# rfonod/geo-trax

Measured on AMD Instinct MI355X. Metric: 4K frames/sec through detect+stabilize+track, higher is better.
Workload: dtype f32 (split-f16x3 MFMA)

## Files before the change

geo-trax_amd/csrc/det_kernels.hip:

```cpp
#include <hip/hip_runtime.h>

#include <mutex>
#include <hip/hip_fp16.h>

#include <cmath>

#include "det_kernels.hpp"

namespace gtx {

typedef _Float16 half8 __attribute__((ext_vector_type(8)));
typedef _Float16 half4 __attribute__((ext_vector_type(4)));

namespace {
inline double py_round(double v) { return std::nearbyint(v); }
}

Letterbox letterbox_geometry(int src_h, int src_w, int imgsz, bool rect, int stride) {
  Letterbox lb{};
  lb.src_h = src_h;
  lb.src_w = src_w;
  const double r = std::min((double)imgsz / src_h, (double)imgsz / src_w);
  lb.new_w = (int)py_round(src_w * r);
  lb.new_h = (int)py_round(src_h * r);
// ... 884 lines not shown
      const float hw = b.z / 2.f, hh = b.w / 2.f;
      reinterpret_cast<float4*>(nb.cand_box)[o] = make_float4(b.x - hw, b.y - hh, b.x + hw, b.y + hh);
    }
  }
}

template <typename T>
__global__ __launch_bounds__(256) void head_raw_kernel(const HeadParams hp, float* __restrict__ out, int logits) {
  const int n = blockIdx.y;
  const int lane = threadIdx.x & 63;
  const int a = (blockIdx.x * blockDim.x + threadIdx.x) >> 6;
  if (a >= hp.n_anchors) return;
  const int l = find_level(hp, a);
  const HeadLevel& L = hp.lv[l];
  const int la = a - L.anchor_begin;
  const T* f = static_cast<const T*>(L.feat) + ((size_t)n * L.h * L.w + la) * L.cstride;
  const float4 b = anchor_box<T>(L, f, la, lane);
  float* o = out + ((size_t)n * hp.n_anchors + a) * (4 + hp.nc);
  if (lane == 0) { o[0] = b.x; o[1] = b.y; o[2] = b.z; o[3] = b.w; }
  const T* fc = f + L.cb;
  for (int c = lane; c < hp.nc; c += 64) {
    float acc = L.bc[c];
    for (int k = 0; k < L.cc; ++k) acc = fmaf(ldf(fc + k), L.wc[c * L.cc + k], acc);
    o[4 + c] = logits ? acc : 1.f / (1.f + expf(-acc));
  }
}

void launch_head_candidates(int dtype, const HeadParams& hp, int n, const NmsBuffers& nb, hipStream_t s) {
  launch_head_gate(dtype, hp, n, nb, s);
  launch_head_boxes(dtype, hp, n, nb, s);
}

void launch_head_gate(int dtype, const HeadParams& hp, int n, const NmsBuffers& nb, hipStream_t s) {
  GTX_HIP(hipMemsetAsync(nb.count, 0, sizeof(int) * n, s));
  if (nb.lvl_count) GTX_HIP(hipMemsetAsync(nb.lvl_count, 0, sizeof(int) * n * kMaxLevels, s));
  dim3 grid(cdiv(hp.n_anchors, 16), n), block(256);
  if (dtype == DT_F16) hipLaunchKernelGGL(head_candidates_kernel<_Float16>, grid, block, 0, s, hp, nb);
  else hipLaunchKernelGGL(head_candidates_kernel<float>, grid, block, 0, s, hp, nb);
  GTX_HIP(hipGetLastError());
}

void launch_head_boxes(int dtype, const HeadParams& hp, int n, const NmsBuffers& nb, hipStream_t s) {
  dim3 grid2(64, n), block(256);
  const size_t lds = (size_t)hp.n_levels * hp.lv[0].cb * 64 * sizeof(float);
  GTX_CHECK(hp.n_levels <= kMaxLevels && hp.lv[0].cb <= 128, "head: %d levels of %d box channels", hp.n_levels, hp.lv[0].cb);
  static std::once_flag once;
  std::call_once(once, [] {
    GTX_HIP(hipFuncSetAttribute(reinterpret_cast<const void*>(head_boxes_kernel<_Float16>), hipFuncAttributeMaxDynamicSharedMemorySize, kMaxLevels * 128 * 64 * 4));
    GTX_HIP(hipFuncSetAttribute(reinterpret_cast<const void*>(head_boxes_kernel<float>), hipFuncAttributeMaxDynamicSharedMemorySize, kMaxLevels * 128 * 64 * 4));
  });
  if (dtype == DT_F16) hipLaunchKernelGGL(head_boxes_kernel<_Float16>, grid2, block, lds, s, hp, nb);
  else hipLaunchKernelGGL(head_boxes_kernel<float>, grid2, block, lds, s, hp, nb);
  GTX_HIP(hipGetLastError());
}

void launch_head_raw(int dtype, const HeadParams& hp, int n, float* out, bool logits, hipStream_t s) {
  dim3 grid(cdiv(hp.n_anchors * 64, 256), n), block(256);
  if (dtype == DT_F16) hipLaunchKernelGGL(head_raw_kernel<_Float16>, grid, block, 0, s, hp, out, logits ? 1 : 0);
  else hipLaunchKernelGGL(head_raw_kernel<float>, grid, block, 0, s, hp, out, logits ? 1 : 0);
  GTX_HIP(hipGetLastError());
}

constexpr int kSmallNms = 4096;
constexpr int kSmallKeep = 2048;

__global__ __launch_bounds__(256) void nms_rank_kernel(const NmsBuffers nb, int limit, float cls_offset) {
  __shared__ float s_sc[256];
  __shared__ int s_an[256];
// ... 146 lines not shown
    if (slot >= nb.max_det) continue;
    float4 b = boxes[i];
    b.x = (b.x - padx) / gain; b.y = (b.y - pady) / gain;
    b.z = (b.z - padx) / gain; b.w = (b.w - pady) / gain;
    b.x = fminf(fmaxf(b.x, 0.f), fw); b.z = fminf(fmaxf(b.z, 0.f), fw);
    b.y = fminf(fmaxf(b.y, 0.f), fh); b.w = fminf(fmaxf(b.w, 0.f), fh);
    float* r = rows + (size_t)slot * 6;
    r[0] = b.x; r[1] = b.y; r[2] = b.z; r[3] = b.w;
    r[4] = nb.s_score[(size_t)n * nb.nms_cap + i];
    r[5] = (float)nb.s_cls[(size_t)n * nb.nms_cap + i];
    if (nb.out_anchor) nb.out_anchor[(size_t)n * nb.max_det + slot] = nb.s_anchor[(size_t)n * nb.nms_cap + i];
  }
}


__device__ __forceinline__ bool iou_gt(const float4& a, float area_a, const float4& b, float thr) {
  const float iw = fminf(a.z, b.z) - fmaxf(a.x, b.x);
  const float ih = fminf(a.w, b.w) - fmaxf(a.y, b.y);
  if (!(iw > 0.f && ih > 0.f)) return false;
  const float area_b = (b.z - b.x) * (b.w - b.y);
  const float inter = iw * ih;
  return inter / (area_a + area_b - inter) > thr;
}

__global__ __launch_bounds__(1024) void nms_small_kernel(const NmsBuffers nb, float thr, float cls_offset, float gain, float padx,
                                                         float pady, float fw, float fh) {
  __shared__ unsigned long long s_key[kSmallNms];
  __shared__ float4 s_box[kSmallNms];
  __shared__ float4 s_kbox[kSmallKeep];
  __shared__ int s_nkeep, s_done;
  const int n = blockIdx.x;
  const int tid = threadIdx.x, lane = tid & 63;
  const int wave = __builtin_amdgcn_readfirstlane(tid >> 6), nwaves = blockDim.x >> 6;
  const int cnt = min(nb.count[n], nb.cap);
  if (cnt > kSmallNms || nb.max_det > kSmallKeep) {
    if (tid == 0) nb.out_n[n] = 0;
    return;
  }
  if (tid == 0) { nb.sorted_n[n] = 0; s_nkeep = 0; s_done = 0; }
  const size_t base = (size_t)n * nb.cap;
  int P = 64;
  while (P < cnt) P <<= 1;
  for (int i = tid; i < P; i += blockDim.x) {
    unsigned long long k = 0ull;
    if (i < cnt) {
      const unsigned sb = __float_as_uint(nb.cand_score[base + i]);
      k = ((unsigned long long)sb << 32) | ((unsigned long long)(0x7FFFFu - (unsigned)nb.cand_anchor[base + i]) << 12) | (unsigned)i;
    }
    s_key[i] = k;
  }
  __syncthreads();
  for (int k = 2; k <= P; k <<= 1)
    for (int j = k >> 1; j > 0; j >>= 1) {
      for (int t = tid; t < P / 2; t += blockDim.x) {
        const int lo = ((t / j) * 2 * j) + (t % j), hi = lo + j;
        const bool desc = ((lo & k) == 0);
        const unsigned long long a = s_key[lo], b = s_key[hi];
        if ((a < b) == desc) { s_key[lo] = b; s_key[hi] = a; }
      }
      __syncthreads();
    }
  for (int i = tid; i < cnt; i += blockDim.x) {
    const int slot = (int)(s_key[i] & 0xFFFu);
    float4 b = reinterpret_cast<const float4*>(nb.cand_box)[base + slot];
    const float o = cls_offset * (float)nb.cand_cls[base + slot];
    b.x += o; b.y += o; b.z += o; b.w += o;
    s_box[i] = b;
// ... 132 lines not shown
```

geo-trax_amd/csrc/det_kernels.hpp:

```cpp
#pragma once
#include <vector>

#include "common.hpp"
#include "conv_igemm.hpp"

namespace gtx {

struct Letterbox {
  int src_h, src_w;
  int net_h, net_w;
  int new_h, new_w;
  int top, left;
  double gain;
};
Letterbox letterbox_geometry(int src_h, int src_w, int imgsz, bool rect, int stride);

void launch_preprocess(int dtype, const uint8_t* frames, int n, const Letterbox& lb, void* img,
                       uint8_t* gray, int gh, int gw, hipStream_t s);

void launch_stem(int dtype, const void* img, int n, int h, int w, const float* w27, const float* bias,
                 const void* wpk_f16, int c0, void* out, int ho, int wo, hipStream_t s, float acc_scale = 1.f);
std::vector<uint16_t> pack_stem_weights_f16(const float* w27, int c0);
std::vector<uint16_t> pack_stem_weights_split(const float* w27, int c0, float* acc_scale);

// ... 14 lines not shown
  float stride;
  int anchor_begin;
};
struct HeadParams {
  HeadLevel lv[kMaxLevels];
  int n_levels;
  int n_anchors;
  int nc;
  float conf;
  unsigned long long class_mask[2];
};

struct NmsBuffers {
  int cap;
  int* count;
  float* cand_score;
  int* cand_anchor;
  int* cand_cls;
  float* cand_box;
  int nms_cap;
  int* sorted_n;
  float* s_box;
  float* s_score;
  int* s_cls;
  int* s_anchor;
  unsigned long long* mask;
  int max_det;
  int* out_n;
  float* out_rows;
  int* out_anchor;
  int* lvl_count;
  int* lvl_list;
  int lvl_cap;
};

struct FeatLevels {
  const void* feat[kMaxLevels];
  int h[kMaxLevels], w[kMaxLevels], cstride[kMaxLevels], coff[kMaxLevels], c[kMaxLevels];
  int anchor_begin[kMaxLevels];
  int n_levels;
  int dim;
};
void launch_obj_feats(int dtype, const FeatLevels& fl, int n, const NmsBuffers& nb, float* out, hipStream_t s);

void launch_head_candidates(int dtype, const HeadParams& hp, int n, const NmsBuffers& nb, hipStream_t s);
void launch_head_gate(int dtype, const HeadParams& hp, int n, const NmsBuffers& nb, hipStream_t s);
void launch_head_boxes(int dtype, const HeadParams& hp, int n, const NmsBuffers& nb, hipStream_t s);

struct SparseBoxLevel {
  const void* in;
  int H, W, cstride, coff, cin;
  const void* w1; const float* b1; float sc1;
  const void* w2; const float* b2; float sc2;
  int anchor_begin;
  const float* wb; const float* bb; float stride;
};
struct SparseBox {
  SparseBoxLevel lv[kMaxLevels];
  int n_levels;
  int cap;
  int* sat_flag;
};
void launch_head_sparse_box(const SparseBox& sb, int n, const NmsBuffers& nb, hipStream_t s);
constexpr int kV10Keep = 300;
void launch_v10_select(int dtype, const HeadParams& hp, int n, const NmsBuffers& cand, const NmsBuffers& sel, float* scores, hipStream_t s);
void launch_v10_rows(const NmsBuffers& sel, const unsigned long long class_mask[2], int n, const Letterbox& lb, hipStream_t s);
// ... 7 lines not shown
```

geo-trax_amd/csrc/detector.cpp:

```cpp
#include "detector.hpp"
#include "split_format.hpp"

#include <algorithm>
#include <cmath>

namespace gtx {

Detector::Detector(gtx_ctx* ctx, const gtx_det_config& cfg)
    : DetectorBase(ctx, cfg, cfg.half ? DT_F16 : (cfg.fp32_split ? DT_F32S : DT_F32), dtype_size(cfg.half ? DT_F16 : DT_F32),
                   cfg.half ? DT_F16 : DT_F32),
      trunk_(*this, ops_, cfg.half ? DT_F16 : DT_F32) {
  dtype_ = cfg.half ? DT_F16 : DT_F32;
  es_ = dtype_size(dtype_);
  lb_ = letterbox_geometry(cfg.frame_h, cfg.frame_w, cfg.imgsz, cfg.rect != 0, 32);
  GTX_CHECK(lb_.net_h % 32 == 0 && lb_.net_w % 32 == 0, "network input %dx%d is not stride aligned", lb_.net_h, lb_.net_w);
}

Detector::~Detector() {
  if (h_feats_) (void)hipHostFree(h_feats_);
  if (h_count_) (void)hipHostFree(h_count_);
}

std::unique_ptr<NetRuntime> Detector::make_exact() const {
  gtx_det_config c = cfg_;
  c.fp32_split = 0;
  return std::unique_ptr<NetRuntime>(new Detector(ctx_, c));
}

View Detector::head_conv(const std::string& name, const View& x, const View* out_slice) {
  ConvArgs a;
  a.out_slice = out_slice;
  a.plain_out = fmt_ == DT_F32S && plain_out_;
  a.force_kc = force_kc_; a.force_bn = force_bn_;
  return emit_named_conv(ops_, name, x, a);
}

void Detector::build_graph() {
  const int H = lb_.net_h, W = lb_.net_w;
  img_ = new_view(H, W, 4);
  alloc_sat_flag();
  const YoloTrunk::Levels trunk = trunk_.build(img_);
  const std::vector<View>& lvl_in = trunk.in;
  const std::vector<float>& strides = trunk.strides;
  det_pfx_ = trunk.det_pfx;
  const int nl = (int)lvl_in.size();
  GTX_CHECK(nl <= kMaxLevels, "internal: %d Detect levels", nl);
  const bool has_o2o = has(det_pfx_ + ".one2one_cv2.0.0.conv.weight");
  end2end_ = cfg_.end2end != 0;
  GTX_CHECK(!end2end_ || has_o2o, "end2end: the checkpoint has no one-to-one head (%s.one2one_cv2 / one2one_cv3): only a YOLOv10 file has", det_pfx_.c_str());
  GTX_CHECK(!end2end_ || !cfg_.obj_feats, "end2end: obj_feats (ReID `model: auto`) is not implemented for the one-to-one head");
  const std::string box_br = end2end_ ? ".one2one_cv2." : ".cv2.", cls_br = end2end_ ? ".one2one_cv3." : ".cv3.";
  GTX_CHECK(has(det_pfx_ + box_br + "0.0.conv.weight") && has(det_pfx_ + cls_br + "0.2.weight"),
            "%s: the checkpoint holds no %s / %s tensors (a fused YOLOv10 export keeps the one-to-one head only: run it with end2end)", det_pfx_.c_str(),
            box_br.substr(1, box_br.size() - 2).c_str(), cls_br.substr(1, cls_br.size() - 2).c_str());

  std::vector<Op> st1, st2;
  const bool dw_cls = trunk.dw_cls;
  std::vector<Op> dw_a, pw_a, dw_b;
  head_ = HeadParams{};
  head_.n_levels = nl;
  head_.nc = cfg_.nc;
  head_.conf = cfg_.conf;
  head_.class_mask[0] = head_.class_mask[1] = cfg_.n_classes == 0 ? ~0ull : 0ull;
  for (int i = 0; i < cfg_.n_classes; ++i)
    if (cfg_.classes[i] >= 0 && cfg_.classes[i] < 128) head_.class_mask[cfg_.classes[i] >> 6] |= 1ull << (cfg_.classes[i] & 63);
  int anchor = 0;
  for (int l = 0; l < nl; ++l) {
    const std::string b2 = det_pfx_ + box_br + std::to_string(l), b3 = det_pfx_ + cls_br + std::to_string(l);
    const HostTensor &w20 = tensor(b2 + ".0.conv.weight"), &w30 = tensor(b3 + (dw_cls ? ".1.1.conv.weight" : ".0.conv.weight"));
    const int cb = (int)w20.shape[0], cc = (int)w30.shape[0], cin = (int)w20.shape[1];
    GTX_CHECK(cin == lvl_in[l].c && (dw_cls || (int)w30.shape[1] == cin), "Detect level %d input channels", l);
    Op o1, o2, o3;
    View h2;
// ... 261 lines not shown
  }
}

void Detector::prime_pad_skip() {
  if (pad_skip_rows_ == 0) return;
  const int N = cfg_.max_batch;
  hipStream_t s = ctx_->stream;
  DevBuf blank;
  blank.alloc((size_t)N * cfg_.frame_h * cfg_.frame_w * 3);
  GTX_HIP(hipMemsetAsync(blank.p, 0, blank.bytes, s));
  pad_skip_on_ = false;
  cur_nb_ = 0;
  set_batch(N);
  launch_preprocess(dtype_, (const uint8_t*)blank.p, N, lb_, img_.ptr, nullptr, cfg_.frame_h / 2, cfg_.frame_w / 2, s);
  for (const Op& op : ops_) run_op(op, N, s);
  int sat = 0;
  if (sat_dev_) GTX_HIP(hipMemcpyAsync(&sat, sat_dev_, sizeof(int), hipMemcpyDeviceToHost, s));
  GTX_HIP(hipStreamSynchronize(s));
  cur_nb_ = 0;
  if (sat_dev_) GTX_HIP(hipMemsetAsync(sat_dev_, 0, sizeof(int), s));
  if (sat) {
    pad_skip_on_ = false;
    pad_skip_rows_ = 0;
    for (Op& op : ops_)
      for (int i = 0; i < kMaxGroup; ++i) op.ty_first[i] = op.ty_count[i] = 0;
    return;
  }
  pad_skip_on_ = true;
}

void Detector::finalize() {
  GTX_CHECK(!finalized_, "finalize called twice");
  GTX_HIP(hipSetDevice(ctx_->device));
  build_graph();
  trunk_.fuse();
  const int N = cfg_.max_batch;
  alloc_outputs();
  nms_ = NmsBuffers{};
  nms_.cap = head_.n_anchors;
  nms_.nms_cap = 30016;
  nms_.max_det = cfg_.max_det;
  nms_.count = (int*)alloc(sizeof(int) * N);
  nms_.cand_score = (float*)alloc(sizeof(float) * N * nms_.cap);
  nms_.cand_anchor = (int*)alloc(sizeof(int) * N * nms_.cap);
  nms_.cand_cls = (int*)alloc(sizeof(int) * N * nms_.cap);
  nms_.cand_box = (float*)alloc(sizeof(float) * 4 * N * nms_.cap);
  if (!end2end_) {
    nms_.sorted_n = (int*)alloc(sizeof(int) * N);
    nms_.s_box = (float*)alloc(sizeof(float) * 4 * N * nms_.nms_cap);
    nms_.s_score = (float*)alloc(sizeof(float) * N * nms_.nms_cap);
    nms_.s_cls = (int*)alloc(sizeof(int) * N * nms_.nms_cap);
    nms_.mask = (unsigned long long*)alloc(sizeof(unsigned long long) * N * (size_t)nms_.nms_cap * (nms_.nms_cap / 64));
  }
  nms_.out_n = (int*)alloc(sizeof(int) * N);
  nms_.out_rows = (float*)alloc(sizeof(float) * 6 * N * cfg_.max_det);
  nms_.s_anchor = nms_.out_anchor = nullptr;
  if (cfg_.obj_feats) {
    nms_.s_anchor = (int*)alloc(sizeof(int) * N * nms_.nms_cap);
    nms_.out_anchor = (int*)alloc(sizeof(int) * N * cfg_.max_det);
    d_feats_ = (float*)alloc(sizeof(float) * N * cfg_.max_det * feat_levels_.dim);
    GTX_HIP(hipHostMalloc((void**)&h_feats_, sizeof(float) * N * cfg_.max_det * feat_levels_.dim));
  }
  if (sparse_on_ && !end2end_) {
    sparse_.cap = kSparseCap;
    sparse_.sat_flag = sat_dev_;
    nms_.lvl_cap = kSparseCap;
    nms_.lvl_count = (int*)alloc(sizeof(int) * N * kMaxLevels);
    nms_.lvl_list = (int*)alloc(sizeof(int) * N * kMaxLevels * kSparseCap);
  }
  if (end2end_) {
    sel_ = nms_;
    sel_.cap = kSelCap;
    sel_.count = (int*)alloc(sizeof(int) * N);
    sel_.cand_score = (float*)alloc(sizeof(float) * N * kSelCap);
    sel_.cand_anchor = (int*)alloc(sizeof(int) * N * kSelCap);
    sel_.cand_cls = (int*)alloc(sizeof(int) * N * kSelCap);
    sel_.cand_box = (float*)alloc(sizeof(float) * 4 * N * kSelCap);
    sel_.lvl_count = sel_.lvl_list = nullptr;
    sel_.lvl_cap = 0;
    if (sparse_on_) {
      sparse_.cap = kSelCap;
      sparse_.sat_flag = sat_dev_;
      sel_.lvl_cap = kSelCap;
      sel_.lvl_count = (int*)alloc(sizeof(int) * N * kMaxLevels);
      sel_.lvl_list = (int*)alloc(sizeof(int) * N * kMaxLevels * kSelCap);
    }
    v10_scores_ = (float*)alloc(sizeof(float) * N * kV10Keep * cfg_.nc);
  }
  GTX_HIP(hipHostMalloc((void**)&h_count_, sizeof(int) * N));
  drop_tensors_unless_fallback();
  if (env_flag("GTX_PAD_SKIP", true)) {
    plan_pad_skip();
    prime_pad_skip();
  }
  set_batch(1);
  GTX_HIP(hipStreamSynchronize(ctx_->stream));
  finalized_ = true;
}

void Detector::run_op(const Op& op, int nb, hipStream_t s) { trunk_.run_op(op, nb, s); }

void Detector::run_post(int nb, hipStream_t s) {
  if (end2end_) {
    HeadParams gate = head_;
    gate.class_mask[0] = gate.class_mask[1] = ~0ull;
    launch_head_gate(dtype_, gate, nb, nms_, s);
    launch_v10_select(dtype_, head_, nb, nms_, sel_, v10_scores_, s);
    if (sparse_on_) {
      launch_head_sparse_box(sparse_, nb, sel_, s);
      dense_head_valid_ = false;
    } else {
      launch_head_boxes(dtype_, head_, nb, sel_, s);
    }
    launch_v10_rows(sel_, head_.class_mask, nb, lb_, s);
    GTX_HIP(hipMemcpyAsync(h_count_, nms_.count, sizeof(int) * nb, hipMemcpyDeviceToHost, s));
    GTX_HIP(hipMemcpyAsync(h_out_n_, sel_.out_n, sizeof(int) * nb, hipMemcpyDeviceToHost, s));
    GTX_HIP(hipMemcpyAsync(h_out_rows_, sel_.out_rows, sizeof(float) * 6 * nb * cfg_.max_det, hipMemcpyDeviceToHost, s));
    if (sat_dev_) GTX_HIP(hipMemcpyAsync(h_sat_, sat_dev_, sizeof(int), hipMemcpyDeviceToHost, s));
    return;
  }
  if (sparse_on_) {
    launch_head_gate(dtype_, head_, nb, nms_, s);
    launch_head_sparse_box(sparse_, nb, nms_, s);
    dense_head_valid_ = false;
  } else {
    launch_head_candidates(dtype_, head_, nb, nms_, s);
  }
  GTX_HIP(hipMemcpyAsync(h_count_, nms_.count, sizeof(int) * nb, hipMemcpyDeviceToHost, s));
  launch_nms(nms_, nb, cfg_.iou, cfg_.agnostic_nms != 0, 30000, lb_, s, 1);
  GTX_HIP(hipMemcpyAsync(h_out_n_, nms_.out_n, sizeof(int) * nb, hipMemcpyDeviceToHost, s));
  GTX_HIP(hipMemcpyAsync(h_out_rows_, nms_.out_rows, sizeof(float) * 6 * nb * cfg_.max_det, hipMemcpyDeviceToHost, s));
  if (sat_dev_) GTX_HIP(hipMemcpyAsync(h_sat_, sat_dev_, sizeof(int), hipMemcpyDeviceToHost, s));
  if (cfg_.obj_feats) {
    launch_obj_feats(fmt_, feat_levels_, nb, nms_, d_feats_, s);
    GTX_HIP(hipMemcpyAsync(h_feats_, d_feats_, sizeof(float) * nb * cfg_.max_det * feat_levels_.dim, hipMemcpyDeviceToHost, s));
  }
}

void Detector::run_dense_box(hipStream_t s) {
  if (!sparse_on_ || dense_head_valid_) return;
  GTX_CHECK(cur_nb_ > 0, "no forward pass has run yet");
  for (Op o : dense_box_ops_) {
    for (int i = 0; i < o.grp.count; ++i) o.grp.p[i].N = cur_nb_;
    conv_group_finalize(o.grp, o.cfg);
    run_op(o, cur_nb_, s);
  }
  dense_head_valid_ = true;
}

void Detector::after_pass(int nb) {
  if (end2end_) return;
  bool over = false, big = false;
  for (int b = 0; b < nb; ++b) {
    over = over || (sparse_on_ && h_count_[b] > kSparseCap);
    big = big || !nms_small_covers(std::min(h_count_[b], nms_.cap), nms_.max_det);
  }
  if (over || big) {
    hipStream_t s = ctx_->stream;
    NmsBuffers dense = nms_;
    if (over) {
      run_dense_box(s);
      launch_head_boxes(dtype_, head_, nb, dense, s);
      ++sparse_overflows_;
    }
    launch_nms(dense, nb, cfg_.iou, cfg_.agnostic_nms != 0, 30000, lb_, s, over ? 0 : 2);
    GTX_HIP(hipMemcpyAsync(h_out_n_, nms_.out_n, sizeof(int) * nb, hipMemcpyDeviceToHost, s));
    GTX_HIP(hipMemcpyAsync(h_out_rows_, nms_.out_rows, sizeof(float) * 6 * nb * cfg_.max_det, hipMemcpyDeviceToHost, s));
    if (cfg_.obj_feats) {
      launch_obj_feats(fmt_, feat_levels_, nb, nms_, d_feats_, s);
      GTX_HIP(hipMemcpyAsync(h_feats_, d_feats_, sizeof(float) * nb * cfg_.max_det * feat_levels_.dim, hipMemcpyDeviceToHost, s));
    }
    record_post_end(s);
    GTX_HIP(hipStreamSynchronize(s));
  }
  if (cfg_.obj_feats) {
    c_feat_n_.assign(cfg_.max_batch, 0);
    c_feats_.resize((size_t)cfg_.max_batch * cfg_.max_det * feat_levels_.dim);
    for (int b = 0; b < nb; ++b) {
      c_feat_n_[b] = h_out_n_[b];
      const size_t o = (size_t)b * cfg_.max_det * feat_levels_.dim;
      memcpy(c_feats_.data() + o, h_feats_ + o, sizeof(float) * h_out_n_[b] * feat_levels_.dim);
    }
  }
}

void Detector::features(int b, float* out, int cap, int* n, int* dim) const {
  GTX_CHECK(cfg_.obj_feats && h_feats_, "features: the detector was created without gtx_det_config.obj_feats");
  GTX_CHECK(b >= 0 && b < cfg_.max_batch, "features: image %d of %d", b, cfg_.max_batch);
  const int cnt = std::min(b < (int)c_feat_n_.size() ? c_feat_n_[b] : 0, cap);
  if (n) *n = cnt;
  if (dim) *dim = feat_levels_.dim;
  if (out && cnt > 0) memcpy(out, c_feats_.data() + (size_t)b * cfg_.max_det * feat_levels_.dim, sizeof(float) * cnt * feat_levels_.dim);
}

void Detector::raw_output(int b, float* out, int* n_anchors, bool logits) {
  GTX_CHECK(finalized_ && cur_nb_ > 0 && b >= 0 && b < cur_nb_, "raw_output: no forward pass for slot %d", b);
  const size_t per = (size_t)head_.n_anchors * (4 + head_.nc);
  if (raw_.bytes < per * cur_nb_ * sizeof(float)) raw_.alloc(per * cur_nb_ * sizeof(float));
  GTX_CHECK(!in_flight_, "raw_output while a batch is in flight: call collect first");
  run_dense_box(ctx_->stream);
  launch_head_raw(dtype_, head_, cur_nb_, raw_.as<float>(), logits, ctx_->stream);
  GTX_HIP(hipMemcpyAsync(out, raw_.as<float>() + per * b, per * sizeof(float), hipMemcpyDeviceToHost, ctx_->stream));
  GTX_HIP(hipStreamSynchronize(ctx_->stream));
  if (n_anchors) *n_anchors = head_.n_anchors;
// ... 24 lines not shown
```

geo-trax_amd/csrc/detector.hpp:

```cpp
#pragma once
#include <map>
#include <memory>
#include <set>
#include <string>
#include <vector>

#include "yolo_trunk.hpp"

namespace gtx {

class Detector : public DetectorBase {
 public:
  Detector(gtx_ctx* ctx, const gtx_det_config& cfg);
  ~Detector() override;
  void finalize() override;
  void raw_output(int b, float* out, int* n_anchors, bool logits = false) override;
  void layer_output(int b, const std::string& layer, float* out, int* h, int* w, int* c) override;
  void features(int b, float* out, int cap, int* n, int* dim) const override;
  void pad_skip(int* on, int* skipped, int* total) const override {
    if (on) *on = (!exact_ && pad_skip_on_) ? 1 : 0;
    if (skipped) *skipped = pad_skip_rows_;
    if (total) *total = pad_skip_total_;
  }
  void sparse_box(int* on, int* overflows) const override {
// ... 8 lines not shown
  std::unique_ptr<NetRuntime> make_exact() const override;
  void release_graph() override { ops_.clear(); trunk_.clear(); }
  View head_conv(const std::string& name, const View& x, const View* out_slice);
  void build_graph();
  void run_op(const Op& op, int nb, hipStream_t s);
  void run_post(int nb, hipStream_t s) override;
  void after_pass(int nb) override;
  void set_batch(int nb) override;

  int dtype_;
  size_t es_;
  std::vector<Op> ops_;
  YoloTrunk trunk_;
  int force_kc_ = 0;
  int force_bn_ = 0;

  HeadParams head_{};
  NmsBuffers nms_{};
  bool end2end_ = false;
  NmsBuffers sel_{};
  float* v10_scores_ = nullptr;
  static constexpr int kSelCap = 304;
  DevBuf raw_;
  bool plain_out_ = false;
  FeatLevels feat_levels_{};
  static constexpr int kSparseCap = 8192;
  bool sparse_on_ = false;
  SparseBox sparse_{};
  Op head_ops_[kMaxLevels][3];
  std::string det_pfx_ = "model.22";
  std::vector<Op> dense_box_ops_;
  bool dense_head_valid_ = false;
  int* h_count_ = nullptr;
  int sparse_overflows_ = 0;
  void run_dense_box(hipStream_t s);
  bool pad_skip_on_ = false;
  int pad_skip_rows_ = 0, pad_skip_total_ = 0;
  void plan_pad_skip();
  void prime_pad_skip();
  float* d_feats_ = nullptr;
  float* h_feats_ = nullptr;
  std::vector<float> c_feats_;
  std::vector<int> c_feat_n_;
};

}
```

geo-trax_amd/csrc/net_runtime.cpp:

```cpp
#include "net_runtime.hpp"
#include "split_format.hpp"

#include <array>
#include <deque>
#include <functional>
#include <mutex>

namespace gtx {

void KernelTable::add(const std::string& label, int n, float t, double f, double b) {
  auto it = idx.find(label);
  size_t k;
  if (it == idx.end()) {
    k = names.size();
    idx[label] = k;
    names.push_back(label);
    launches.push_back(0); ms.push_back(0.f); flops.push_back(0.0); bytes.push_back(0.0);
  } else {
    k = it->second;
  }
  launches[k] += n;
  ms[k] += t;
  flops[k] += f;
  bytes[k] += b;
}

NetRuntime::~NetRuntime() {
  if (h_sat_) (void)hipHostFree(h_sat_);
}

void NetRuntime::set_tensor(const std::string& name, const float* data, int ndim, const int64_t* shape) {
  GTX_CHECK(!finalized_, "set_tensor after finalize");
  HostTensor t;
  size_t n = 1;
  for (int i = 0; i < ndim; ++i) {
    t.shape.push_back(shape[i]);
    n *= (size_t)shape[i];
  }
  t.data.assign(data, data + n);
  tensors_[name] = std::move(t);
}

const HostTensor& NetRuntime::tensor(const std::string& name) const {
  auto it = tensors_.find(name);
  if (it == tensors_.end()) fail(-1, "missing tensor '%s'", name.c_str());
  return it->second;
}

const float* NetRuntime::bias_of(const std::string& name, int cout) const {
  if (!has(name + ".bias")) return nullptr;
  const HostTensor& b = tensor(name + ".bias");
  GTX_CHECK((int)b.data.size() == cout, "%s: bias size", name.c_str());
  return b.data.data();
}

void* NetRuntime::alloc(size_t bytes) {
  bufs_.emplace_back(bytes);
  GTX_HIP(hipMemset(bufs_.back().p, 0, bufs_.back().bytes));
  return bufs_.back().p;
}

// ... 127 lines not shown
  p.in_cstride = x.cstride; p.in_coff = x.coff;
  p.out_cstride = out.cstride; p.out_coff = out.coff;
  p.res_cstride = a.residual ? a.residual->cstride : 0;
  p.res_coff = a.residual ? a.residual->coff : 0;
  p.act = a.act;
  p.acc_scale = pw->acc_scale;
  p.out_plain = (fmt_ == DT_F32S && out.plain) ? 1 : 0;
  p.sat_flag = fmt_ == DT_F32S ? sat_dev_ : nullptr;
  return out;
}

void NetRuntime::read_view(const View& v, int slot, float* out) const {
  const size_t px = (size_t)v.h * v.w;
  const size_t es = (fmt_ == DT_F16 && !v.plain) ? 2 : 4;
  std::vector<uint8_t> host(px * v.cstride * es);
  GTX_HIP(hipMemcpy(host.data(), (const uint8_t*)v.ptr + (size_t)slot * px * v.cstride * es, host.size(), hipMemcpyDeviceToHost));
  for (size_t p = 0; p < px; ++p)
    for (int k = 0; k < v.c; ++k) {
      const size_t src = p * v.cstride + v.coff + k;
      float f;
      if (fmt_ == DT_F32S && !v.plain) {
        f = pair_element(host.data(), src);
      } else if (es == 2) {
        _Float16 hv;
        memcpy(&hv, host.data() + src * 2, 2);
        f = (float)hv;
      } else {
        memcpy(&f, host.data() + src * 4, 4);
      }
      out[p * v.c + k] = f;
    }
}

void NetRuntime::alloc_sat_flag() {
  if (fmt_ != DT_F32S) return;
  sat_dev_ = (int*)alloc(sizeof(int));
  GTX_HIP(hipHostMalloc((void**)&h_sat_, sizeof(int)));
  *h_sat_ = 0;
}

void NetRuntime::drop_tensors_unless_fallback() {
  static const bool fallback = env_flag("GTX_SAT_FALLBACK", true);
  if (fmt_ != DT_F32S || !fallback) tensors_.clear();
}

bool NetRuntime::saturated(bool clear) {
  const bool r = sat_seen_;
  if (clear) {
    sat_seen_ = false;
    if (sat_dev_ && !exact_) {
      GTX_HIP(hipSetDevice(ctx_->device));
      GTX_HIP(hipMemsetAsync(sat_dev_, 0, sizeof(int), ctx_->stream));
    }
  }
  return r;
}

void NetRuntime::fall_back_to_exact() {
  std::unique_ptr<NetRuntime> d = make_exact();
  for (const auto& kv : tensors_) d->set_tensor(kv.first, kv.second.data.data(), (int)kv.second.shape.size(), kv.second.shape.data());
  d->finalize();
  GTX_HIP(hipStreamSynchronize(ctx_->stream));
  release_graph();
  layer_views_.clear();
  bufs_.clear();
  tensors_.clear();
  exact_ = std::move(d);
}


DetectorBase::DetectorBase(gtx_ctx* ctx, const gtx_det_config& cfg, int fmt, size_t view_es, int in_dtype)
    : NetRuntime(ctx, fmt, view_es, std::max(cfg.max_batch, 1)), cfg_(cfg), in_dtype_(in_dtype) {
  GTX_CHECK(cfg.imgsz > 0 && cfg.imgsz % 32 == 0, "imgsz must be a positive multiple of 32 (got %d)", cfg.imgsz);
  GTX_CHECK(cfg.max_det > 0 && cfg.nc > 0 && cfg.nc <= 128, "max_det must be positive and nc in [1, 128] (got %d, %d)", cfg.max_det, cfg.nc);
  GTX_CHECK(cfg.frame_h > 0 && cfg.frame_w > 0, "frame size must be given");
  cfg_.max_batch = max_batch_;
  GTX_HIP(hipSetDevice(ctx->device));
  for (auto& e : ev_) GTX_HIP(hipEventCreateWithFlags(&e, wait_event_flags(true)));
  for (auto& e : ev_up_) GTX_HIP(hipEventCreate(&e));
}

DetectorBase::~DetectorBase() {
  if (h_out_n_) (void)hipHostFree(h_out_n_);
  if (h_out_rows_) (void)hipHostFree(h_out_rows_);
  for (auto& e : ev_)
    if (e) (void)hipEventDestroy(e);
  for (auto& e : ev_up_)
    if (e) (void)hipEventDestroy(e);
  for (auto& e : trace_ev_)
    if (e) (void)hipEventDestroy(e);
}

void DetectorBase::alloc_outputs() {
  const int N = cfg_.max_batch;
  gray_h_ = cfg_.frame_h / 2;
  gray_w_ = cfg_.frame_w / 2;
  gray_.alloc((size_t)kGrayRing * N * gray_h_ * gray_w_);
  GTX_HIP(hipHostMalloc((void**)&h_out_n_, sizeof(int) * N));
  GTX_HIP(hipHostMalloc((void**)&h_out_rows_, sizeof(float) * 6 * N * cfg_.max_det));
}

void DetectorBase::submit_dev(const void* frames, int nb, int h, int w) {
  GTX_CHECK(finalized_, "detector not finalized");
  GTX_CHECK(!in_flight_, "submit while a batch is in flight: call collect first");
  GTX_CHECK(nb >= 1 && nb <= cfg_.max_batch, "batch %d outside [1,%d]", nb, cfg_.max_batch);
  GTX_CHECK(h == cfg_.frame_h && w == cfg_.frame_w, "frame is %dx%d, detector was created for %dx%d", w, h, cfg_.frame_w, cfg_.frame_h);
  GTX_HIP(hipSetDevice(ctx_->device));
  hipStream_t s = ctx_->stream;
  set_batch(nb);
  cur_frames_ = frames;
  gray_slot_ = (gray_slot_ + 1) % kGrayRing;
  uint8_t* gray = gray_.as<uint8_t>() + (size_t)gray_slot_ * cfg_.max_batch * gray_h_ * gray_w_;
  GTX_HIP(hipEventRecord(ev_[0], s));
  launch_preprocess(in_dtype_, (const uint8_t*)frames, nb, lb_, img_.ptr, gray, gray_h_, gray_w_, s);
  GTX_HIP(hipEventRecord(ev_[1], s));
  flight_traced_ = trace_every_ > 0 && (trace_count_++ % trace_every_) == 0;
  run_ops(nb, s, flight_traced_ ? trace_ev_.data() : nullptr);
  GTX_HIP(hipEventRecord(ev_[2], s));
  run_post(nb, s);
  GTX_HIP(hipEventRecord(ev_[3], s));
  in_flight_ = true;
  flight_nb_ = nb;
}

void DetectorBase::collect(int* n_out, float* xyxy, float* conf, int* cls, float speed_ms[3]) {
  GTX_CHECK(in_flight_, "collect without a submitted batch");
  GTX_HIP(hipSetDevice(ctx_->device));
  GTX_HIP(hipEventSynchronize(ev_[3]));
  in_flight_ = false;
  collected_gray_slot_ = gray_slot_;
// ... 107 lines not shown
```

geo-trax_amd/csrc/net_runtime.hpp:

```cpp
#pragma once
#include <map>
#include <memory>
#include <string>
#include <vector>

#include "../../include/gtx.h"
#include "common.hpp"
#include "conv_igemm.hpp"
#include "det_kernels.hpp"

struct gtx_ctx {
  int device = 0;
  hipStream_t stream = nullptr;
  hipDeviceProp_t prop{};
  ~gtx_ctx() {
    if (stream) (void)hipStreamDestroy(stream);
  }
};

namespace gtx {

struct HostTensor {
  std::vector<int64_t> shape;
  std::vector<float> data;
// ... 68 lines not shown
  };
  template <class OpT>
  View emit_conv(std::vector<OpT>& ops, const std::string& name, const float* w_oihw, int cout, int cin, int ks, const float* bias,
                 const View& x, const ConvArgs& a) {
    OpT op;
    op.kind = OpT::CONV;
    op.name = name;
    const View out = conv_problem(name, w_oihw, cout, cin, ks, bias, x, a, op.cfg, op.grp.p[0]);
    op.grp.count = 1;
    op.family = conv_kernel_name(op.cfg);
    ops.push_back(op);
    layer_views_[name] = out;
    return out;
  }
  template <class OpT>
  View emit_named_conv(std::vector<OpT>& ops, const std::string& name, const View& x, ConvArgs a) {
    const HostTensor& w = tensor(name + ".weight");
    GTX_CHECK(w.shape.size() == 4 && w.shape[2] == w.shape[3], "%s: expected OIHW square kernel", name.c_str());
    const int cout = (int)w.shape[0], cin = (int)w.shape[1], ks = (int)w.shape[2];
    a.out_pixels = (long)x.n * ((x.h + 2 * (ks / 2) - ks) / a.stride + 1) * ((x.w + 2 * (ks / 2) - ks) / a.stride + 1);
    return emit_conv(ops, name, w.data.data(), cout, cin, ks, bias_of(name, cout), x, a);
  }
  virtual void conv_config_rule(const std::string& name, ConvConfig& cfg) const { (void)name; (void)cfg; }

  void set_layer_view(const std::string& name, const View& v) { layer_views_[name] = v; }
  void repoint_layer_views(const void* from, void* to);
  size_t release_buffer(const void* p);
  int format() const { return fmt_; }
  int device() const { return ctx_->device; }
  int* sat_flag() const { return sat_dev_; }

  void read_view(const View& v, int slot, float* out) const;

  void alloc_sat_flag();
  void drop_tensors_unless_fallback();
  bool can_fall_back() const { return !tensors_.empty(); }
  virtual std::unique_ptr<NetRuntime> make_exact() const = 0;
  virtual void release_graph() = 0;
  void fall_back_to_exact();
  template <class T> T* live_as() { return exact_ ? static_cast<T*>(exact_.get()) : static_cast<T*>(this); }

  gtx_ctx* ctx_;
  int fmt_;
  size_t view_es_;
  int max_batch_;
  bool finalized_ = false;
  int cur_nb_ = 0;
  std::map<std::string, HostTensor> tensors_;
  std::vector<DevBuf> bufs_;
  std::map<std::string, View> layer_views_;
  std::unique_ptr<NetRuntime> exact_;
  int* sat_dev_ = nullptr;
  int* h_sat_ = nullptr;
  bool sat_seen_ = false;

 private:
  View conv_problem(const std::string& name, const float* w_oihw, int cout, int cin, int ks, const float* bias, const View& x,
                    const ConvArgs& a, ConvConfig& cfg, ConvProblem& p);
};

template <class F>
void NetRuntime::time_ops(int nb, int iters, F fold) {
  hipStream_t s = ctx_->stream;
  set_batch(nb);
  const size_t n = op_count();
  std::vector<hipEvent_t> ev(n + 1);
  for (auto& e : ev) GTX_HIP(hipEventCreate(&e));
  for (int it = 0; it < iters; ++it) {
    run_ops(nb, s, ev.data());
    GTX_HIP(hipStreamSynchronize(s));
    for (size_t i = 0; i < n; ++i) {
      float t = 0.f;
      GTX_HIP(hipEventElapsedTime(&t, ev[i], ev[i + 1]));
      fold(i, t);
    }
  }
  for (auto& e : ev) (void)hipEventDestroy(e);
}

class DetectorBase : public NetRuntime {
 public:
  DetectorBase(gtx_ctx* ctx, const gtx_det_config& cfg, int fmt, size_t view_es, int in_dtype);
  ~DetectorBase() override;
  DetectorBase* live() { return live_as<DetectorBase>(); }
  void input_size(int* h, int* w) const { *h = lb_.net_h; *w = lb_.net_w; }
  void detect_dev(const void* frames, int nb, int h, int w, int* n_out, float* xyxy, float* conf, int* cls, float speed_ms[3]);
  void submit_dev(const void* frames, int nb, int h, int w);
  void collect(int* n_out, float* xyxy, float* conf, int* cls, float speed_ms[3]);
  void detect_host(const uint8_t* frame, int h, int w, int* n_out, float* xyxy, float* conf, int* cls, float speed_ms[3]);
  const void* gray(int b, int* gh, int* gw) const;
  virtual void raw_output(int b, float* out, int* n_anchors, bool logits = false) = 0;
  virtual void layer_output(int b, const std::string& layer, float* out, int* h, int* w, int* c) = 0;
  void profile(int nb, int iters, std::vector<std::string>& names, std::vector<int>& launches, std::vector<float>& ms,
               std::vector<double>& flops, std::vector<double>& bytes);
  void set_trace(int every_n);
  void trace_report(std::vector<std::string>& names, std::vector<int>& launches, std::vector<float>& ms, std::vector<double>& flops,
                    std::vector<double>& bytes);
  virtual void features(int b, float* out, int cap, int* n, int* dim) const = 0;
  virtual void pad_skip(int* on, int* skipped, int* total) const = 0;
  virtual void sparse_box(int* on, int* overflows) const = 0;

  static constexpr int kGrayRing = 16;

 protected:
  void alloc_outputs();
  virtual void run_post(int nb, hipStream_t s) = 0;
  virtual void after_pass(int nb) { (void)nb; }
  void record_post_end(hipStream_t s) { GTX_HIP(hipEventRecord(ev_[3], s)); }

  gtx_det_config cfg_;
  int in_dtype_;
  Letterbox lb_{};
  View img_;
  int* h_out_n_ = nullptr;
  float* h_out_rows_ = nullptr;
  bool in_flight_ = false;
  int flight_nb_ = 0;

 private:
  DevBuf frame_stage_;
  DevBuf gray_;
  int gray_h_ = 0, gray_w_ = 0;
  int gray_slot_ = 0, collected_gray_slot_ = 0;
  const void* cur_frames_ = nullptr;
  hipEvent_t ev_[4]{};
  hipEvent_t ev_up_[2]{};
  int trace_every_ = 0, trace_count_ = 0;
  bool flight_traced_ = false;
  std::vector<hipEvent_t> trace_ev_;
  std::vector<double> trace_ms_;
  std::vector<int> trace_n_;
  std::vector<double> trace_flops_, trace_bytes_;
};

}

struct gtx_detector {
  std::unique_ptr<gtx::DetectorBase> impl;
};
```

Baseline: 1189.

## Pack post-processing outputs into one record buffer and copy it once

Places the saturation flag, candidate counts, output counts and output rows in one contiguous device record, which is fetched with a single device-to-host copy instead of three or four small ones. The per-frame memsets of the candidate counters are removed. The NMS kernel now snapshots the raw count into the record and resets the counters itself for the next pass. The dense fallback path has to restore and clear the counters by hand, which adds coupling and ordering risk between kernels.

```diff
diff --git a/geo-trax_amd/csrc/det_kernels.hip b/geo-trax_amd/csrc/det_kernels.hip
--- a/geo-trax_amd/csrc/det_kernels.hip
+++ b/geo-trax_amd/csrc/det_kernels.hip
@@ -940,8 +940,10 @@
 }
 
 void launch_head_gate(int dtype, const HeadParams& hp, int n, const NmsBuffers& nb, hipStream_t s) {
-  GTX_HIP(hipMemsetAsync(nb.count, 0, sizeof(int) * n, s));
-  if (nb.lvl_count) GTX_HIP(hipMemsetAsync(nb.lvl_count, 0, sizeof(int) * n * kMaxLevels, s));
+  if (!nb.rec_count) {
+    GTX_HIP(hipMemsetAsync(nb.count, 0, sizeof(int) * n, s));
+    if (nb.lvl_count) GTX_HIP(hipMemsetAsync(nb.lvl_count, 0, sizeof(int) * n * kMaxLevels, s));
+  }
   dim3 grid(cdiv(hp.n_anchors, 16), n), block(256);
   if (dtype == DT_F16) hipLaunchKernelGGL(head_candidates_kernel<_Float16>, grid, block, 0, s, hp, nb);
   else hipLaunchKernelGGL(head_candidates_kernel<float>, grid, block, 0, s, hp, nb);
@@ -1154,7 +1156,17 @@
   const int n = blockIdx.x;
   const int tid = threadIdx.x, lane = tid & 63;
   const int wave = __builtin_amdgcn_readfirstlane(tid >> 6), nwaves = blockDim.x >> 6;
-  const int cnt = min(nb.count[n], nb.cap);
+  const int raw = nb.count[n];
+  const int cnt = min(raw, nb.cap);
+  if (nb.rec_count) {
+    __syncthreads();
+    if (tid == 0) {
+      nb.rec_count[n] = raw;
+      nb.count[n] = 0;
+      if (nb.lvl_count)
+        for (int l = 0; l < kMaxLevels; ++l) nb.lvl_count[n * kMaxLevels + l] = 0;
+    }
+  }
   if (cnt > kSmallNms || nb.max_det > kSmallKeep) {
     if (tid == 0) nb.out_n[n] = 0;
     return;
diff --git a/geo-trax_amd/csrc/det_kernels.hpp b/geo-trax_amd/csrc/det_kernels.hpp
--- a/geo-trax_amd/csrc/det_kernels.hpp
+++ b/geo-trax_amd/csrc/det_kernels.hpp
@@ -70,6 +70,7 @@
   int* lvl_count;
   int* lvl_list;
   int lvl_cap;
+  int* rec_count;
 };
 
 struct FeatLevels {
diff --git a/geo-trax_amd/csrc/detector.cpp b/geo-trax_amd/csrc/detector.cpp
--- a/geo-trax_amd/csrc/detector.cpp
+++ b/geo-trax_amd/csrc/detector.cpp
@@ -18,7 +18,8 @@
 
 Detector::~Detector() {
   if (h_feats_) (void)hipHostFree(h_feats_);
-  if (h_count_) (void)hipHostFree(h_count_);
+  if (h_rec_) (void)hipHostFree(h_rec_);
+  else if (h_count_) (void)hipHostFree(h_count_);
 }
 
 std::unique_ptr<NetRuntime> Detector::make_exact() const {
@@ -38,7 +39,7 @@
 void Detector::build_graph() {
   const int H = lb_.net_h, W = lb_.net_w;
   img_ = new_view(H, W, 4);
-  alloc_sat_flag();
+  alloc_sat_flag(d_rec_, h_rec_);
   const YoloTrunk::Levels trunk = trunk_.build(img_);
   const std::vector<View>& lvl_in = trunk.in;
   const std::vector<float>& strides = trunk.strides;
@@ -366,15 +367,23 @@
 void Detector::finalize() {
   GTX_CHECK(!finalized_, "finalize called twice");
   GTX_HIP(hipSetDevice(ctx_->device));
+  const int N = cfg_.max_batch;
+  if (env_flag("GTX_POST_RECORD", true)) {
+    rec_head_ = (1 + 2 * N + 3) & ~3;
+    const size_t bytes = sizeof(int) * ((size_t)rec_head_ + (size_t)6 * N * cfg_.max_det);
+    d_rec_ = (int*)alloc(bytes);
+    GTX_HIP(hipHostMalloc((void**)&h_rec_, bytes));
+    memset(h_rec_, 0, bytes);
+  }
   build_graph();
   trunk_.fuse();
-  const int N = cfg_.max_batch;
-  alloc_outputs();
+  alloc_outputs(h_rec_ ? h_rec_ + 1 + N : nullptr, h_rec_ ? reinterpret_cast<float*>(h_rec_ + rec_head_) : nullptr);
   nms_ = NmsBuffers{};
   nms_.cap = head_.n_anchors;
   nms_.nms_cap = 30016;
   nms_.max_det = cfg_.max_det;
-  nms_.count = (int*)alloc(sizeof(int) * N);
+  nms_.rec_count = (d_rec_ && !end2end_) ? d_rec_ + 1 : nullptr;
+  nms_.count = (d_rec_ && end2end_) ? d_rec_ + 1 : (int*)alloc(sizeof(int) * N);
   nms_.cand_score = (float*)alloc(sizeof(float) * N * nms_.cap);
   nms_.cand_anchor = (int*)alloc(sizeof(int) * N * nms_.cap);
   nms_.cand_cls = (int*)alloc(sizeof(int) * N * nms_.cap);
@@ -386,8 +395,8 @@
     nms_.s_cls = (int*)alloc(sizeof(int) * N * nms_.nms_cap);
     nms_.mask = (unsigned long long*)alloc(sizeof(unsigned long long) * N * (size_t)nms_.nms_cap * (nms_.nms_cap / 64));
   }
-  nms_.out_n = (int*)alloc(sizeof(int) * N);
-  nms_.out_rows = (float*)alloc(sizeof(float) * 6 * N * cfg_.max_det);
+  nms_.out_n = d_rec_ ? d_rec_ + 1 + N : (int*)alloc(sizeof(int) * N);
+  nms_.out_rows = d_rec_ ? reinterpret_cast<float*>(d_rec_ + rec_head_) : (float*)alloc(sizeof(float) * 6 * N * cfg_.max_det);
   nms_.s_anchor = nms_.out_anchor = nullptr;
   if (cfg_.obj_feats) {
     nms_.s_anchor = (int*)alloc(sizeof(int) * N * nms_.nms_cap);
@@ -421,7 +430,8 @@
     }
     v10_scores_ = (float*)alloc(sizeof(float) * N * kV10Keep * cfg_.nc);
   }
-  GTX_HIP(hipHostMalloc((void**)&h_count_, sizeof(int) * N));
+  if (h_rec_) h_count_ = h_rec_ + 1;
+  else GTX_HIP(hipHostMalloc((void**)&h_count_, sizeof(int) * N));
   drop_tensors_unless_fallback();
   if (env_flag("GTX_PAD_SKIP", true)) {
     plan_pad_skip();
@@ -433,6 +443,10 @@
 }
 
 void Detector::run_op(const Op& op, int nb, hipStream_t s) { trunk_.run_op(op, nb, s); }
+
+void Detector::copy_record(int nb, hipStream_t s) {
+  GTX_HIP(hipMemcpyAsync(h_rec_, d_rec_, sizeof(int) * ((size_t)rec_head_ + (size_t)6 * nb * cfg_.max_det), hipMemcpyDeviceToHost, s));
+}
 
 void Detector::run_post(int nb, hipStream_t s) {
   if (end2end_) {
@@ -447,6 +461,7 @@
       launch_head_boxes(dtype_, head_, nb, sel_, s);
     }
     launch_v10_rows(sel_, head_.class_mask, nb, lb_, s);
+    if (d_rec_) return copy_record(nb, s);
     GTX_HIP(hipMemcpyAsync(h_count_, nms_.count, sizeof(int) * nb, hipMemcpyDeviceToHost, s));
     GTX_HIP(hipMemcpyAsync(h_out_n_, sel_.out_n, sizeof(int) * nb, hipMemcpyDeviceToHost, s));
     GTX_HIP(hipMemcpyAsync(h_out_rows_, sel_.out_rows, sizeof(float) * 6 * nb * cfg_.max_det, hipMemcpyDeviceToHost, s));
@@ -460,11 +475,15 @@
   } else {
     launch_head_candidates(dtype_, head_, nb, nms_, s);
   }
-  GTX_HIP(hipMemcpyAsync(h_count_, nms_.count, sizeof(int) * nb, hipMemcpyDeviceToHost, s));
+  if (!d_rec_) GTX_HIP(hipMemcpyAsync(h_count_, nms_.count, sizeof(int) * nb, hipMemcpyDeviceToHost, s));
   launch_nms(nms_, nb, cfg_.iou, cfg_.agnostic_nms != 0, 30000, lb_, s, 1);
-  GTX_HIP(hipMemcpyAsync(h_out_n_, nms_.out_n, sizeof(int) * nb, hipMemcpyDeviceToHost, s));
-  GTX_HIP(hipMemcpyAsync(h_out_rows_, nms_.out_rows, sizeof(float) * 6 * nb * cfg_.max_det, hipMemcpyDeviceToHost, s));
-  if (sat_dev_) GTX_HIP(hipMemcpyAsync(h_sat_, sat_dev_, sizeof(int), hipMemcpyDeviceToHost, s));
+  if (d_rec_) {
+    copy_record(nb, s);
+  } else {
+    GTX_HIP(hipMemcpyAsync(h_out_n_, nms_.out_n, sizeof(int) * nb, hipMemcpyDeviceToHost, s));
+    GTX_HIP(hipMemcpyAsync(h_out_rows_, nms_.out_rows, sizeof(float) * 6 * nb * cfg_.max_det, hipMemcpyDeviceToHost, s));
+    if (sat_dev_) GTX_HIP(hipMemcpyAsync(h_sat_, sat_dev_, sizeof(int), hipMemcpyDeviceToHost, s));
+  }
   if (cfg_.obj_feats) {
     launch_obj_feats(fmt_, feat_levels_, nb, nms_, d_feats_, s);
     GTX_HIP(hipMemcpyAsync(h_feats_, d_feats_, sizeof(float) * nb * cfg_.max_det * feat_levels_.dim, hipMemcpyDeviceToHost, s));
@@ -492,6 +511,10 @@
   if (over || big) {
     hipStream_t s = ctx_->stream;
     NmsBuffers dense = nms_;
+    if (nms_.rec_count) {
+      GTX_HIP(hipMemcpyAsync(nms_.count, h_count_, sizeof(int) * nb, hipMemcpyHostToDevice, s));
+      dense.rec_count = nullptr;
+    }
     if (over) {
       run_dense_box(s);
       launch_head_boxes(dtype_, head_, nb, dense, s);
@@ -504,6 +527,7 @@
       launch_obj_feats(fmt_, feat_levels_, nb, nms_, d_feats_, s);
       GTX_HIP(hipMemcpyAsync(h_feats_, d_feats_, sizeof(float) * nb * cfg_.max_det * feat_levels_.dim, hipMemcpyDeviceToHost, s));
     }
+    if (nms_.rec_count) GTX_HIP(hipMemsetAsync(nms_.count, 0, sizeof(int) * nb, s));
     record_post_end(s);
     GTX_HIP(hipStreamSynchronize(s));
   }
diff --git a/geo-trax_amd/csrc/detector.hpp b/geo-trax_amd/csrc/detector.hpp
--- a/geo-trax_amd/csrc/detector.hpp
+++ b/geo-trax_amd/csrc/detector.hpp
@@ -64,6 +64,10 @@
   std::vector<Op> dense_box_ops_;
   bool dense_head_valid_ = false;
   int* h_count_ = nullptr;
+  int* d_rec_ = nullptr;
+  int* h_rec_ = nullptr;
+  int rec_head_ = 0;
+  void copy_record(int nb, hipStream_t s);
   int sparse_overflows_ = 0;
   void run_dense_box(hipStream_t s);
   bool pad_skip_on_ = false;
diff --git a/geo-trax_amd/csrc/net_runtime.cpp b/geo-trax_amd/csrc/net_runtime.cpp
--- a/geo-trax_amd/csrc/net_runtime.cpp
+++ b/geo-trax_amd/csrc/net_runtime.cpp
@@ -26,7 +26,7 @@
 }
 
 NetRuntime::~NetRuntime() {
-  if (h_sat_) (void)hipHostFree(h_sat_);
+  if (h_sat_ && own_h_sat_) (void)hipHostFree(h_sat_);
 }
 
 void NetRuntime::set_tensor(const std::string& name, const float* data, int ndim, const int64_t* shape) {
@@ -220,10 +220,16 @@
     }
 }
 
-void NetRuntime::alloc_sat_flag() {
+void NetRuntime::alloc_sat_flag(int* dev, int* host) {
   if (fmt_ != DT_F32S) return;
-  sat_dev_ = (int*)alloc(sizeof(int));
-  GTX_HIP(hipHostMalloc((void**)&h_sat_, sizeof(int)));
+  if (dev) {
+    sat_dev_ = dev;
+    h_sat_ = host;
+    own_h_sat_ = false;
+  } else {
+    sat_dev_ = (int*)alloc(sizeof(int));
+    GTX_HIP(hipHostMalloc((void**)&h_sat_, sizeof(int)));
+  }
   *h_sat_ = 0;
 }
 
@@ -269,8 +275,8 @@
 }
 
 DetectorBase::~DetectorBase() {
-  if (h_out_n_) (void)hipHostFree(h_out_n_);
-  if (h_out_rows_) (void)hipHostFree(h_out_rows_);
+  if (h_out_n_ && own_h_out_) (void)hipHostFree(h_out_n_);
+  if (h_out_rows_ && own_h_out_) (void)hipHostFree(h_out_rows_);
   for (auto& e : ev_)
     if (e) (void)hipEventDestroy(e);
   for (auto& e : ev_up_)
@@ -279,11 +285,17 @@
     if (e) (void)hipEventDestroy(e);
 }
 
-void DetectorBase::alloc_outputs() {
+void DetectorBase::alloc_outputs(int* h_out_n, float* h_out_rows) {
   const int N = cfg_.max_batch;
   gray_h_ = cfg_.frame_h / 2;
   gray_w_ = cfg_.frame_w / 2;
   gray_.alloc((size_t)kGrayRing * N * gray_h_ * gray_w_);
+  if (h_out_n) {
+    h_out_n_ = h_out_n;
+    h_out_rows_ = h_out_rows;
+    own_h_out_ = false;
+    return;
+  }
   GTX_HIP(hipHostMalloc((void**)&h_out_n_, sizeof(int) * N));
   GTX_HIP(hipHostMalloc((void**)&h_out_rows_, sizeof(float) * 6 * N * cfg_.max_det));
 }
diff --git a/geo-trax_amd/csrc/net_runtime.hpp b/geo-trax_amd/csrc/net_runtime.hpp
--- a/geo-trax_amd/csrc/net_runtime.hpp
+++ b/geo-trax_amd/csrc/net_runtime.hpp
@@ -124,7 +124,7 @@
 
   void read_view(const View& v, int slot, float* out) const;
 
-  void alloc_sat_flag();
+  void alloc_sat_flag(int* dev = nullptr, int* host = nullptr);
   void drop_tensors_unless_fallback();
   bool can_fall_back() const { return !tensors_.empty(); }
   virtual std::unique_ptr<NetRuntime> make_exact() const = 0;
@@ -144,6 +144,7 @@
   std::unique_ptr<NetRuntime> exact_;
   int* sat_dev_ = nullptr;
   int* h_sat_ = nullptr;
+  bool own_h_sat_ = true;
   bool sat_seen_ = false;
 
  private:
@@ -195,7 +196,7 @@
   static constexpr int kGrayRing = 16;
 
  protected:
-  void alloc_outputs();
+  void alloc_outputs(int* h_out_n = nullptr, float* h_out_rows = nullptr);
   virtual void run_post(int nb, hipStream_t s) = 0;
   virtual void after_pass(int nb) { (void)nb; }
   void record_post_end(hipStream_t s) { GTX_HIP(hipEventRecord(ev_[3], s)); }
@@ -206,6 +207,7 @@
   View img_;
   int* h_out_n_ = nullptr;
   float* h_out_rows_ = nullptr;
+  bool own_h_out_ = true;
   bool in_flight_ = false;
   int flight_nb_ = 0;
 
```

After: 1193 (median of 4 runs). About the same (+0.3%).
